# Gustavroot/DeflatedMLMC_Schwinger

Measured on AMD Instinct MI355X. Metric: hutchinson_probe_samples_per_sec_schwinger128, higher is better.
Workload: dtype f64

## Files before the change

deflatedmlmc_schwinger_amd/csrc/sw_engine.hip:

```cpp
#include "../../include/schwinger_hip.h"
#include "sw_kernels.hpp"
#include "sw_pack.hpp"
#include "sw_poly.hpp"

#include <dlfcn.h>

#include <algorithm>
#include <chrono>
#include <cmath>
#include <complex>
#include <cstdarg>
#include <cstdio>
#include <cstdlib>
#include <cstring>
#include <functional>
#include <map>
#include <mutex>
#include <string>
#include <type_traits>
#include <vector>

using swk::cplx;
using swk::cplxf;
using swk::PtrList;
// ... 149 lines not shown
  bool eo_skew_chunk = false;
  bool gram_cycle = true;
  bool eo_product = true;
  int gj_block = 32;
  int eo_tile = 0;
  int dense_lds = 4;
  int eo_tile_dbg = 0;
  int num_cus = 256;
  bool direct_small = true;
  bool lgmres_aug = true;
  bool stencil_nt = false;
  int stencil_tile = 0;
  int stencil_spw = 0;
  bool cgs2 = false;
  bool verify = true;
  bool inner_cgs2 = false;
  bool pyth_last = true;
  bool eo_solve = true;
  bool eo_direct = true;
  bool precond_f32 = false;
  int kd = 0;
  cplx* U = nullptr;
  int defl_gemm = 0;
  int lkd[SW_MAX_LEVELS] = {0};
  cplx* lV[SW_MAX_LEVELS] = {nullptr};
  int* perm_src[SW_MAX_LEVELS] = {nullptr};
  EllOp rhsmap[SW_MAX_LEVELS];
  cplx* partial = nullptr;
  size_t partial_bytes = 0;
  cplx* small = nullptr;
  size_t small_bytes = 0;
  void* stage = nullptr;
  size_t stage_bytes = 0;
  std::vector<std::pair<void*, size_t>> allocs;
  int pb_level = -1, pb_nb = 0, pb_nbp = 0;
  int8_t* pb_probes = nullptr;
  struct ProbeSlot {
    int8_t* p = nullptr;
    size_t bytes = 0;
    int level = -1, nb = 0;
    hipEvent_t ready = nullptr;
    bool pending = false;
  };
  std::vector<ProbeSlot> slots;
  bool mt_set = false;
  uint32_t* mt_win0 = nullptr;
  uint32_t* mt_win = nullptr;
  int mt_cur = 0;
  uint64_t mt_pos = 0;
  uint32_t* mt_poly = nullptr;
  uint64_t mt_dist = 0;
  uint32_t* mt_family = nullptr;
  uint64_t mt_fam_seg = 0;
  int mt_fam_count = 0;
  cplx *pb_x0 = nullptr, *pb_rhs = nullptr, *pb_z = nullptr, *pb_xc = nullptr, *pb_xc2 = nullptr,
       *pb_y = nullptr, *pb_w = nullptr, *pb_w2 = nullptr, *pb_xd = nullptr;
  int pb_ws_nbp = 0;
  cplx* pb_est = nullptr;
  int* pb_iters = nullptr;
  std::vector<int32_t> last_iters_f, last_iters_c;
  bool profiling = false;
  std::vector<EventRec> recs;
  std::vector<hipEvent_t> evpool;
  double tacc[T_NCAT] = {0};
  int64_t tcount[T_NCAT] = {0};
  double twork[T_NCAT] = {0};
  int64_t launches = 0;
  int* d_notconv = nullptr;
  int nc_next = 0;
  int* h_notconv = nullptr;
  int* d_tick = nullptr;
  bool fused_reduce = true;
  double stop_factor = 1.0;
  std::vector<double> direct_relres;
  int64_t direct_fallbacks = 0;
  double alloc_s = 0.0, alloc_bytes = 0.0;
  int64_t alloc_calls = 0, pool_hits = 0;
// ... 34 lines not shown
    field<&sw_engine::mfma_small_tiles>("mfma_small_tiles",
                                        [](double v) { return v == 0.0 || v == 2.0 || v == 4.0; },
                                        "mfma_small_tiles must be 0, 2 or 4"),
    field<&sw_engine::mfma3_tiles>("mfma3_tiles",
                                   [](double v) { const int t = (int)v; return t == 0 || t == 1 || t == 2 || t == 4; },
                                   "mfma3_tiles must be 0, 1, 2 or 4"),
    field<&sw_engine::bsr_map>("bsr_map", [](double v) { return (int)v >= 0 && (int)v <= 3; },
                               "bsr_map must be 0..3"),
    field<&sw_engine::dense_map>("dense_map", [](double v) { return (int)v >= 0 && (int)v <= 3; },
                                 "dense_map must be 0..3"),
    field<&sw_engine::bsr_sub>("bsr_sub", [](double v) { return (int)v >= 1; }, "bsr_sub must be >= 1"),
    field<&sw_engine::bsr_stages>("bsr_stages", [](double v) { return v == 2.0 || v == 4.0 || v == 8.0; },
                                  "bsr_stages must be 2, 4 or 8 (dense_stages: or 16)"),
    field<&sw_engine::dense_stages>("dense_stages",
                                    [](double v) { return v == 2.0 || v == 4.0 || v == 8.0 || v == 16.0; },
                                    "dense_stages must be 2, 4 or 8 (dense_stages: or 16)"),
    field<&sw_engine::bsr_nt>("bsr_nt"),
    field<&sw_engine::bsr_xreg>("bsr_xreg"),
    {"dense_lds", get_field<&sw_engine::dense_lds>,
     [](sw_engine* h, double v) { h->dense_lds = v == 1.0 ? 2 : (int)v; },
     [](double v) { return v == 0.0 || v == 1.0 || v == 2.0 || v == 4.0; }, "dense_lds must be 0, 2 or 4"},
    field<&sw_engine::defl_gemm>("defl_gemm", [](double v) { return v == 0.0 || v == 1.0; },
                                 "defl_gemm must be 0 or 1"),
    field<&sw_engine::fused_reduce>("fused_reduce"),
    {"dot_blocks", [](const sw_engine*) { return (double)g_dot_blocks; },
     [](sw_engine*, double v) { g_dot_blocks = g_dot_pmax = std::max(64, (int)v); }},
    field<&sw_engine::gj_block>("gj_block",
                                [](double v) {
                                  const int b = (int)v;
                                  return b == 0 || (b >= 8 && b <= 256 && b % 8 == 0);
                                },
                                "gj_block must be 0 or a multiple of 8 in 8..256"),
    field<&sw_engine::stencil_nt>("stencil_nt"),
    field<&sw_engine::stencil_tile>("stencil_tile"),
    field<&sw_engine::stencil_spw>("stencil_spw",
                                   [](double v) {
                                     const int t = (int)v;
                                     return t == 0 || t == 1 || t == 2 || t == 4 || t == 8;
                                   },
                                   "stencil_spw must be 0,1,2,4,8"),
    field<&sw_engine::eo_tile>("eo_tile", [](double v) { return v == 0.0 || v == 4.0 || v == 8.0; },
                               "eo_tile must be 0 (off), 4 or 8 waves"),
    {"eo_tile_dbg", get_field<&sw_engine::eo_tile_dbg>, [](sw_engine* h, double v) { h->eo_tile_dbg = (int)v & 3; }},
    field<&sw_engine::eo_skew>("eo_skew", [](double v) { return !(v < -1.0 || v > 65536.0); },
                               "eo_skew must be -1 (automatic), 0 (off) or a strip height"),
    field<&sw_engine::eo_skew_chunk>("eo_skew_chunk"),
// ... 597 lines not shown
  int P, rpb;
  row_blocking(n, nbp, nrm_out != nullptr, &P, &rpb);
  const int ngroups = (P + SW_RED_GROUP - 1) / SW_RED_GROUP;
  if (nrm_out) SWCHK(ensure_partial(h, (size_t)(P + ngroups) * nbp * sizeof(cplx)));
  const bool fused = nrm_out && fused_ok(h, P, nbp);
  const swk::RedArgs ra = red_args(h, fused, P, 1, nbp, nrm_out, nullptr, nullptr);
  const swk::FgTail tl = (fused && tail) ? *tail : kNoTail;
  dim3 grid(P, nbp / 64);
  SWCHK(pick_ge<2, 4, 8, 16, 24, 34>(K, [&](auto KT) {
    if (nrm_out)
      return launch(h, T_AXPY, swk::k_multiaxpy<KT, true, CV, CW>, grid, dim3(SW_BLOCK), V, K, coef, sign, Win, Wout,
                    n, nbp, rpb, h->partial, w32, ra, tl);
    return launch(h, T_AXPY, swk::k_multiaxpy<KT, false, CV, CW>, grid, dim3(SW_BLOCK), V, K, coef, sign, Win, Wout,
                  n, nbp, rpb, h->partial, w32, ra, tl);
  }));
  if (nrm_out && !fused) {
    SWCHK(launch(h, T_DOTS, swk::k_reduce_partials, dim3(1, nbp / 64), dim3(SW_BLOCK), h->partial, P, 1, nbp,
                 nrm_out, (const cplx*)nullptr, (cplx*)nullptr));
  }
  if (tail && !fused) SWCHK(launch_tail(h, *tail));
  return 0;
}

static int zero_vec(sw_engine* h, cplx* p, int n, int nbp) {
  LaunchScope ls(h, T_AXPY);
  HIPCHK(hipMemsetAsync(p, 0, (size_t)n * nbp * sizeof(cplx), h->stream));
  return 0;
}
static int copy_vec(sw_engine* h, cplx* dst, const cplx* src, int n, int nbp) {
  LaunchScope ls(h, T_AXPY);
  HIPCHK(hipMemcpyAsync(dst, src, (size_t)n * nbp * sizeof(cplx), hipMemcpyDeviceToDevice,
                        h->stream));
  return 0;
}

static int ensure_small(sw_engine* h, int nbp) {
  const size_t need = (size_t)(SW_MAX_DEFL + 8) * nbp * sizeof(cplx);
  if (h->small_bytes >= need) return 0;
  if (h->small) SWCHK(dev_free(h, h->small));
  h->small = nullptr;
  void* q;
  SWCHK(dev_alloc(h, &q, need));
  h->small = (cplx*)q;
  h->small_bytes = need;
  return 0;
}
// ... 260 lines not shown
    std::vector<int> ord(P.ngroups);
    if (P.order && h->ell_order)
      HIPCHK(hipMemcpy(ord.data(), P.order, ord.size() * sizeof(int), hipMemcpyDeviceToHost));
    else
      for (int g = 0; g < P.ngroups; ++g) ord[g] = g;
    std::vector<int> ev;
    for (int g : ord) {
      const long long row = (long long)g * P.G;
      const bool even = lv.stencil ? (row < lv.n / 2) : (even_row_tile[row / 16] != 0);
      if (even) ev.push_back(g);
    }
    if (ev.empty()) continue;
    SWCHK(upload(h, &P.order_even, ev.data(), ev.size()));
    P.ngroups_even = (int)ev.size();
  }
  H.even_valid = true;
  return 0;
}

static inline int* sink_slot(sw_engine* h);
static bool f32_capable(const Hier& H, int level);

static int gram_cycle(sw_engine* h, const KrylovSys& sys, const cplx* R, cplx* X, int L, KrylovWS& ws, int nbp,
                      swk::FgTail tg) {
  const size_t vec = (size_t)sys.n * nbp;
  PtrList pu, pz;
  pu.p[0] = R;
  for (int j = 0; j < L; ++j) {
    cplx* z = ws.Z + vec * j;
    cplx* w = ws.V + vec * j;
    SWCHK(sys.precond(pu.p[j], z));
    SWCHK(sys.apply(0, z, nullptr, w));
    pu.p[j + 1] = w;
    pz.p[j] = z;
  }
  tg.kind = SW_TAIL_GRAM;
  tg.s = ws.sc;
  tg.j = L;
  tg.h1 = ws.gram;
  SWCHK(multigram(h, pu, L + 1, sys.n, nbp, ws.gram, &tg));
  return multiaxpy(h, pz, L, ws.sc.ys, 1.0, X, X, sys.n, nbp, nullptr);
}

static int kcycle_gram(sw_engine* h, Hier& H, int level, const cplx* B, cplx* X, int L, KrylovWS& ws, int nbp) {
  swk::FgTail tg{};
  tg.first_cycle = 1;
  tg.notconv = sink_slot(h);
  SWCHK(zero_vec(h, X, H.lv[level].n, nbp));
  return gram_cycle(h, full_system(h, H, level, nbp, true, false), B, X, L, ws, nbp, tg);
}

static int coarse_correction(sw_engine* h, Hier& H, int l, int nbp) {
  Level& lv = H.lv[l];
  Level& lc = H.lv[l + 1];
  const int last = H.nlevels - 1;
  if (lv.kcycle > 0 && l + 1 < last) {
    SWCHK(ensure_krylov(h, lc.kws, lv.kcycle, lc.n, nbp, false));
    int P = 0, rpb = 0;
    row_blocking(lc.n, nbp, true, &P, &rpb);
    if (h->gram_cycle && lv.kcycle <= SW_GRAM_MAXL && fused_ok(h, P, nbp) &&
        !(h->precond_f32 && f32_capable(H, l + 1)))
      return kcycle_gram(h, H, l + 1, lc.b, lc.x, lv.kcycle, lc.kws, nbp);
    return fgmres(h, H, l + 1, lc.b, lc.x, 0.0, lv.kcycle, lv.kcycle, false, lc.kws, nbp, nullptr);
  }
// ... 2245 lines not shown
  }
  return s;
}

static int reduced_rhs(sw_engine* h, Level& lv, const cplx* B, KrylovWS& ws, int nbp) {
  PtrList pl;
  pl.p[0] = B;
  const swk::FgTail tbeg = tail_begin(ws, 1);
  SWCHK(multidot(h, pl, 1, B, lv.n, nbp, ws.nrm, nullptr, nullptr, &tbeg));
  return eo_hop<0>(h, lv, B, B, ws.xacc, nbp);
}

static int fgmres_eo(sw_engine* h, Hier& H, const cplx* B, cplx* X, double tol, int maxiter, int m,
                     KrylovWS& ws, int nbp, int* iters_total) {
  Level& lv = H.lv[0];
  SWCHK(ensure_level_ws(h, lv, nbp));
  SWCHK(reduced_rhs(h, lv, B, ws, nbp));
  SWCHK(fgmres_loop(h, H, 0, reduced_system(h, H, nbp), ws.xacc, X, tol, maxiter, m, true, ws, nbp,
                    iters_total));
  return eo_hop<1>(h, lv, B, X, X, nbp);
}

static int fgmres_eo_gram(sw_engine* h, Hier& H, const cplx* B, cplx* X, double tol, int maxiter, int m,
                          KrylovWS& ws, int nbp, int* iters_total) {
  Level& lv = H.lv[0];
  const int hid_idx = (int)(&H - &h->hier[0]);
  const int hint = h->lazy_sync ? h->sync_hint[hid_idx][0] : 0;
  const KrylovSys sys = reduced_system(h, H, nbp);
  const double tol_stop = tol * h->stop_factor;
  SWCHK(ensure_level_ws(h, lv, nbp));
  SWCHK(reset_slots(h));
  SWCHK(reduced_rhs(h, lv, B, ws, nbp));
  const cplx* bp = ws.xacc;
  SWCHK(zero_vec(h, X, sys.n, nbp));
  std::vector<std::complex<double>> hrr(nbp), hrr0(nbp);
  int done = 0;
  bool converged = false;
  const cplx* Rcur = bp;
  int L = std::min(m, maxiter);
  while (done < maxiter && !converged) {
    L = std::max(1, std::min(L, std::min(m, maxiter - done)));
    int* slot = nullptr;
    SWCHK(take_slot(h, &slot));
    swk::FgTail tg{};
    tg.tol = tol;
    tg.tol_stop = tol_stop;
    tg.iter_base = done;
    tg.notconv = slot;
    SWCHK(gram_cycle(h, sys, Rcur, X, L, ws, nbp, tg));
    done += L;
    SWCHK(sys.apply(1, X, bp, ws.rres));
    Rcur = ws.rres;
    const bool observe = tol_stop > 0.0 && (hint <= 0 || done + m >= hint || done >= maxiter);
    int Lnext = m;
    if (observe) {
      int left = 0;
      SWCHK(read_slot(h, slot, &left));
      if (left == 0) {
        converged = true;
      } else {
        HIPCHK(hipMemcpy(hrr.data(), ws.sc.relres, sizeof(cplx) * nbp, hipMemcpyDeviceToHost));
        HIPCHK(hipMemcpy(hrr0.data(), ws.sc.g, sizeof(cplx) * nbp, hipMemcpyDeviceToHost));
        double need = 1.0;
        for (int c = 0; c < nbp; ++c) {
          const double r1 = hrr[c].real(), r0 = hrr0[c].real();
          if (!(r1 >= tol_stop) || !(r0 > 0.0)) continue;
          const double rate = std::pow(std::min(0.9, std::max(1e-6, r1 / r0)), 1.0 / L);
          need = std::max(need, std::ceil(std::log(0.9 * tol_stop / r1) / std::log(rate)));
        }
        Lnext = (int)std::min<double>(m, need);
      }
    }
    if (converged && h->verify) {
      PtrList pr;
      pr.p[0] = ws.rres;
      int* vslot = nullptr;
      SWCHK(take_slot(h, &vslot));
      const swk::FgTail tv = tail_verify(ws, tol, tol_stop, vslot);
      SWCHK(multidot(h, pr, 1, ws.rres, sys.n, nbp, ws.nrm, nullptr, nullptr, &tv));
      int left = 0;
      SWCHK(read_slot(h, vslot, &left));
      if (left != 0) {
        converged = false;
        Lnext = 1;
      }
    }
    L = Lnext;
  }
  SWCHK(eo_hop<1>(h, lv, B, X, X, nbp));
  if (iters_total) *iters_total = done;
  h->sync_hint[hid_idx][0] = converged ? done : 0;
  return 0;
}

static bool level_is_direct(sw_engine* h, Hier& H, int level) {
  return h->direct_small && level < H.nlevels - 1 && !H.lv[level].stencil && H.lv[level].dinv.set &&
         h->use_mfma;
}

static int solve_dev(sw_engine* h, int hid, int level0, const cplx* B, cplx* X, double tol,
                     int maxiter, int nbp, int* total) {
  Hier& H = h->hier[hid];
  Level& lv = H.lv[level0];
  if (level0 == H.nlevels - 1 && H.nlevels > 1) {
    SWCHK(apply_coarsest(h, H, B, X, nbp));
    if (total) *total = 1;
    return 0;
  }
  if (level_is_direct(h, H, level0)) {
    SWCHK(ensure_level_ws(h, lv, nbp));
    SWCHK(launch_bsr(h, lv.dinv, 0, B, nullptr, X, nbp, T_COARSEST, cplx{0.0, 0.0}));
    SWCHK(apply_op(h, lv, 1, X, B, lv.r, nbp));
    SWCHK(launch_bsr(h, lv.dinv, 0, lv.r, nullptr, lv.t, nbp, T_COARSEST, cplx{0.0, 0.0}));
    SWCHK(vec_add(h, X, lv.t, X, lv.n, nbp));
    if (total) *total = 1;
// ... 4 lines not shown
      SWCHK(dot_into(h, lv.r, lv.r, lv.n, nbp, h->small));
      SWCHK(dot_into(h, B, B, lv.n, nbp, h->small + nbp));
      SWCHK(stream_sync(h));
      std::vector<std::complex<double>> nn(2 * (size_t)nbp);
      HIPCHK(hipMemcpy(nn.data(), h->small, sizeof(cplx) * 2 * nbp, hipMemcpyDeviceToHost));
      double worst = 0.0;
      for (int j = 0; j < nbp; ++j) {
        const double b2 = nn[nbp + j].real(), r2 = nn[j].real();
        const double rr = b2 > 0.0 ? std::sqrt(r2 / b2) : 0.0;
        h->direct_relres[j] = rr;
        worst = std::max(worst, rr);
      }
      if (!(worst > tol * h->stop_factor)) return 0;
      if (pass == 3) break;
      SWCHK(launch_bsr(h, lv.dinv, 0, lv.r, nullptr, lv.t, nbp, T_COARSEST, cplx{0.0, 0.0}));
      SWCHK(vec_add(h, X, lv.t, X, lv.n, nbp));
    }
    h->direct_relres.clear();
    h->direct_fallbacks++;
    const int mfb = std::min(h->restart, std::max(1, maxiter));
    SWCHK(ensure_krylov(h, lv.sws, mfb, lv.n, nbp, true));
    return fgmres(h, H, level0, B, X, tol, maxiter, mfb, true, lv.sws, nbp, total);
  }
  const int m = std::min(h->restart, std::max(1, maxiter));
  SWCHK(ensure_krylov(h, lv.sws, m, lv.n, nbp, true));
  if (eo_solve_eligible(h, H, level0)) {
    const bool k32 = h->precond_f32 && h->f32_krylov && f32_capable(H, 0);
    int P = 0, rpb = 0;
    row_blocking(lv.n / 2, nbp, true, &P, &rpb);
    if (h->gram_cycle && !k32 && m <= SW_GRAM_MAXL && fused_ok(h, P, nbp))
      return fgmres_eo_gram(h, H, B, X, tol, maxiter, m, lv.sws, nbp, total);
    return fgmres_eo(h, H, B, X, tol, maxiter, m, lv.sws, nbp, total);
  }
  return fgmres(h, H, level0, B, X, tol, maxiter, m, true, lv.sws, nbp, total);
}

static int fetch_iters(sw_engine* h, KrylovWS& ws, int nb, int32_t* iters, double* relres,
                       int fallback_iters) {
  std::vector<int> it(ws.nbp);
  std::vector<std::complex<double>> rr(ws.nbp);
  HIPCHK(hipMemcpy(it.data(), ws.sc.iters, sizeof(int) * ws.nbp, hipMemcpyDeviceToHost));
  HIPCHK(hipMemcpy(rr.data(), ws.sc.relres, sizeof(cplx) * ws.nbp, hipMemcpyDeviceToHost));
  for (int j = 0; j < nb; ++j) {
    if (iters) iters[j] = it[j] >= 0 ? it[j] : fallback_iters;
    if (relres) relres[j] = rr[j].real();
  }
  return 0;
}

int sw_solve(sw_engine* h, int hid, int level0, int nb, const double* B, double* X, double tol,
             int maxiter, int32_t* iters, double* relres) {
  SWCHK(check_hier(h, hid, level0, true));
  if (nb <= 0 || !B || !X || maxiter < 1) return sw_fail(h, "bad arguments");
  HIPCHK(hipSetDevice(h->device));
  Hier& H = h->hier[hid];
  const int nbp = pad64(nb);
// ... 8 lines not shown
    for (int j = 0; j < nb; ++j) {
      if (iters) iters[j] = 1;
      if (relres) relres[j] = 0.0;
    }
    return 0;
  }
  if (level_is_direct(h, H, level0) && (int)h->direct_relres.size() >= nb) {
    for (int j = 0; j < nb; ++j) {
      if (iters) iters[j] = 1;
      if (relres) relres[j] = h->direct_relres[j];
    }
    return 0;
  }
  return fetch_iters(h, lv.sws, nb, iters, relres, total);
}

static int ensure_probe_ws(sw_engine* h, int nbp) {
  if (h->pb_ws_nbp == nbp && h->pb_x0) return 0;
  Hier& H0 = h->hier[0];
  int nmax = 0;
  for (int l = 0; l < H0.nlevels; ++l) nmax = std::max(nmax, H0.lv[l].n);
  const size_t cnt = (size_t)nmax * nbp;
  SWCHK(dev_realloc(h, &h->pb_x0, cnt));
  SWCHK(dev_realloc(h, &h->pb_rhs, cnt));
  SWCHK(dev_realloc(h, &h->pb_z, cnt));
  SWCHK(dev_realloc(h, &h->pb_xc, cnt));
  SWCHK(dev_realloc(h, &h->pb_xc2, cnt));
  SWCHK(dev_realloc(h, &h->pb_y, cnt));
  SWCHK(dev_realloc(h, &h->pb_w, cnt));
  SWCHK(dev_realloc(h, &h->pb_w2, cnt));
  SWCHK(dev_realloc(h, &h->pb_xd, cnt));
  SWCHK(dev_realloc(h, &h->pb_est, (size_t)4 * nbp));
  SWCHK(dev_realloc(h, &h->pb_iters, (size_t)2 * nbp));
  h->pb_ws_nbp = nbp;
  return 0;
}

int sw_probes_upload_slot(sw_engine* h, int slot, int level, int nb, const int8_t* probes) {
  SWCHK(check_hier(h, 0, level, true));
  if (nb <= 0 || !probes) return sw_fail(h, "bad arguments");
  if (slot < 0 || slot >= 4096) return sw_fail(h, "probe slot %d out of range", slot);
  HIPCHK(hipSetDevice(h->device));
  Level& lv = h->hier[0].lv[level];
  const size_t bytes = (size_t)nb * lv.n;
  if ((int)h->slots.size() <= slot) h->slots.resize(slot + 1);
  sw_engine::ProbeSlot& sl = h->slots[slot];
// ... 166 lines not shown
  return 0;
}

static int deflate(sw_engine* h, const cplx* U, int kd, const int* srcrow, const cplx* X, cplx* out,
                   int n, int nbp) {
  const int ld = defl_ld(kd);
  cplx* cbuf = h->small + 8 * nbp;
  if (h->defl_gemm || kd > 64) {
    const int nchunks = nbp / 16;
    const int pmax = std::max(1, (n + 63) / 64);
    int P = std::max(1, std::min(pmax, 2048 / nchunks));
    const int rpb = (n + P - 1) / P;
    P = (n + rpb - 1) / rpb;
    SWCHK(ensure_partial(h, (size_t)P * ld * nbp * sizeof(cplx)));
    SWCHK(pick_ge<64, 128, 256>(ld, [&](auto LD) {
      return launch(h, T_DEFL, swk::k_defl_gemm_dots<LD / 64>, dim3(P, nchunks), dim3(SW_BLOCK), U, ld, X, n, nbp,
                    rpb, h->partial);
    }));
    SWCHK(launch(h, T_DEFL, swk::k_reduce_partials, dim3(ld, nbp / 64), dim3(SW_BLOCK), h->partial, P, ld, nbp,
                 cbuf, (const cplx*)nullptr, (cplx*)nullptr));
    return launch(h, T_DEFL, swk::k_defl_gemm_apply, dim3((n + 63) / 64, nbp / 64), dim3(SW_BLOCK), U, ld,
                  (const cplx*)cbuf, srcrow, X, out, n, nbp);
  }
  int P, rpb;
  row_blocking(n, nbp, true, &P, &rpb);
  for (int k0 = 0; k0 < kd; k0 += 32) {
    const int kc = std::min(32, kd - k0);
    SWCHK(ensure_partial(h, (size_t)P * kc * nbp * sizeof(cplx)));
    SWCHK(pick_ge<8, 16, 32>(kc, [&](auto KC) {
      return launch(h, T_DEFL, swk::k_defl_dots<KC>, dim3(P, nbp / 64), dim3(SW_BLOCK), (const cplx*)(U + k0), ld,
                    kc, X, n, nbp, rpb, h->partial);
    }));
    SWCHK(launch(h, T_DEFL, swk::k_reduce_partials, dim3(kc, nbp / 64), dim3(SW_BLOCK), h->partial, P, kc, nbp,
                 cbuf + (size_t)k0 * nbp, (const cplx*)nullptr, (cplx*)nullptr));
  }
  {
    dim3 grid((n + SW_WAVES_PER_BLOCK - 1) / SW_WAVES_PER_BLOCK, nbp / 64);
    SWCHK(launch(h, T_DEFL, swk::k_defl_apply, grid, dim3(SW_BLOCK), U, ld, kd, cbuf, srcrow, X, out, n, nbp));
  }
  return 0;
}

int sw_apply_deflation(sw_engine* h, int which, int level, int nb, const double* X, double* Y) {
  SWCHK(check_hier(h, 0, level, false));
  if (which != 0 && which != 1) return sw_fail(h, "which must be 0 (Hutchinson) or 1 (MLMC level)");
  if (which == 0 && level != 0) return sw_fail(h, "the Hutchinson deflation acts at level 0");
  if (nb <= 0 || !X || !Y) return sw_fail(h, "bad arguments");
  const int kd = which == 0 ? h->kd : h->lkd[level];
  const cplx* U = which == 0 ? h->U : h->lV[level];
  if (kd <= 0 || !U) return sw_fail(h, "no deflation vectors registered at level %d", level);
  HIPCHK(hipSetDevice(h->device));
  Level& lv = h->hier[0].lv[level];
  const int nbp = pad64(nb);
  cplx *a, *b;
  SWCHK(io_vectors(h, lv, nbp, &a, &b));
  SWCHK(ensure_small(h, nbp));
  SWCHK(pack_host(h, lv, nb, X, a, nbp));
  SWCHK(deflate(h, U, kd, which == 0 ? (const int*)h->perm_src[0] : nullptr, a, b, lv.n, nbp));
  return unpack_host(h, lv, nb, b, Y, nbp);
}

int sw_hutch_run(sw_engine* h, int mode, int level, double tol, int maxiter) {
  SWCHK(check_hier(h, 0, level, true));
  if (h->pb_level != level || h->pb_nb <= 0) return sw_fail(h, "no probes uploaded for level %d", level);
  if (maxiter < 1) return sw_fail(h, "maxiter must be >= 1");
  HIPCHK(hipSetDevice(h->device));
  Hier& H0 = h->hier[0];
  const int nb = h->pb_nb, nbp = h->pb_nbp;
  Level& lv = H0.lv[level];
  const int n = lv.n;
  SWCHK(ensure_probe_ws(h, nbp));
  SWCHK(ensure_small(h, nbp));
  if (h->pb_slot >= 0 && h->pb_slot < (int)h->slots.size() && h->slots[h->pb_slot].pending) {
    HIPCHK(hipStreamWaitEvent(h->stream, h->slots[h->pb_slot].ready, 0));
    h->slots[h->pb_slot].pending = false;
  }
  SWCHK(launch(h, T_OTHER, swk::k_pack_i8, dim3((n + 63) / 64, nbp / 64), dim3(SW_BLOCK), h->pb_probes, nb, n,
               (const int*)lv.rowmap, h->pb_x0, nbp));
  const int fine_hid = (level == 0 && h->hier[h->solver_hid].ready) ? h->solver_hid : 0;
  if (fine_hid != 0 && h->hier[fine_hid].lv[0].n != n)
    return sw_fail(h, "solver hierarchy level-0 size mismatch");
  if (mode == SW_MODE_HUTCHINSON) {
    if (level != 0) return sw_fail(h, "Hutchinson mode runs at level 0");
    const int kd = h->kd;
    if (kd > 0) {
      SWCHK(deflate(h, h->U, kd, (const int*)h->perm_src[0], h->pb_x0, h->pb_rhs, n, nbp));
    } else {
      dim3 grid((n + SW_WAVES_PER_BLOCK - 1) / SW_WAVES_PER_BLOCK, nbp / 64);
      SWCHK(launch(h, T_DEFL, swk::k_gather_rows, grid, dim3(SW_BLOCK), (const int*)h->perm_src[0], h->pb_x0,
                   h->pb_rhs, n, nbp));
    }
    int total = 0;
    SWCHK(solve_dev(h, fine_hid, 0, h->pb_rhs, h->pb_z, tol, maxiter, nbp, &total));
    SWCHK(dot_into(h, h->pb_x0, h->pb_z, n, nbp, h->pb_est));
    SWCHK(stream_sync(h));
    SWCHK(record_iters(h, &h->hier[fine_hid].lv[0].sws, total, h->last_iters_f, nb));
    h->last_iters_c.assign(nb, 0);
    return 0;
  }
  if (mode == SW_MODE_LEVEL) {
    const cplx* xdef = h->pb_x0;
    if (h->rhsmap[level].set) {
      SWCHK(launch_ell(h, h->rhsmap[level], 0, xdef, nullptr, h->pb_rhs, nbp, T_OTHER));
      xdef = h->pb_rhs;
// ... 275 lines not shown
```

deflatedmlmc_schwinger_amd/csrc/sw_kernels.hpp:

```cpp
#pragma once
#include <hip/hip_runtime.h>
#include <stdint.h>

namespace swk {

typedef double2 cplx;

#define SW_WAVE 64
#define SW_BLOCK 256
#define SW_WAVES_PER_BLOCK 4

__device__ __forceinline__ cplx cmake(double a, double b) { cplx r; r.x = a; r.y = b; return r; }
__device__ __forceinline__ cplx cadd(cplx a, cplx b) { return cmake(a.x + b.x, a.y + b.y); }
__device__ __forceinline__ cplx csub(cplx a, cplx b) { return cmake(a.x - b.x, a.y - b.y); }
__device__ __forceinline__ cplx cmul(cplx a, cplx b) {
  return cmake(fma(a.x, b.x, -a.y * b.y), fma(a.x, b.y, a.y * b.x));
}
__device__ __forceinline__ cplx cmulc(cplx a, cplx b) {
  return cmake(fma(a.x, b.x, a.y * b.y), fma(a.x, b.y, -a.y * b.x));
}
__device__ __forceinline__ void cfma(cplx& acc, cplx a, cplx b) {
  acc.x = fma(a.x, b.x, acc.x);
  acc.x = fma(-a.y, b.y, acc.x);
  acc.y = fma(a.x, b.y, acc.y);
// ... 1404 lines not shown
  const size_t item = (size_t)blockIdx.x * SW_WAVES_PER_BLOCK + (threadIdx.x >> 6);
  if (item >= (size_t)(n >> 4) * KS) return;
  const int rt = (int)(item / KS), ks = (int)(item - (size_t)rt * KS);
  const cplx v = A[((size_t)rt * 16 + (lane & 15)) * n + k0 + 4 * ks + (lane >> 4)];
  vals[item * 64 + lane] = cmake(-v.x, -v.y);
  if (lane == 0) kcol[item] = 4 * ks;
}

__global__ __launch_bounds__(SW_BLOCK) void k_gj_unpermute(cplx* __restrict__ A, int n,
                                                           const int* __restrict__ pivs) {
  const int r = blockIdx.x * SW_BLOCK + threadIdx.x;
  if (r >= n) return;
  cplx* row = A + (size_t)r * n;
  for (int k = n - 1; k >= 0; --k) {
    const int p = pivs[k];
    if (p != k) {
      const cplx t = row[k];
      row[k] = row[p];
      row[p] = t;
    }
  }
}

__global__ __launch_bounds__(SW_BLOCK) void k_pack_i8(const int8_t* __restrict__ src, int nb,
                                                      int n, const int* __restrict__ rowmap,
                                                      cplx* __restrict__ dst, int nbp) {
  __shared__ int8_t tile[64][65];
  const int i0 = blockIdx.x * 64;
  const int j0 = blockIdx.y * 64;
  const int tx = threadIdx.x & 63, ty = threadIdx.x >> 6;
  for (int jj = ty; jj < 64; jj += 4) {
    const int j = j0 + jj, i = i0 + tx;
    tile[jj][tx] = (j < nb && i < n) ? src[(size_t)j * n + i] : (int8_t)0;
  }
  __syncthreads();
  for (int ii = ty; ii < 64; ii += 4) {
    const int i = i0 + ii;
    if (i < n) {
      const size_t row = rowmap ? (size_t)rowmap[i] : (size_t)i;
      const int v = tile[tx][ii];
      dst[row * nbp + j0 + tx] = (v == 2 || v == -2) ? cmake(0.0, (double)(v / 2)) : cmake((double)v, 0.0);
    }
  }
}

__global__ __launch_bounds__(SW_BLOCK) void k_pack_c(const cplx* __restrict__ src, int nb, int n,
                                                     const int* __restrict__ rowmap,
                                                     cplx* __restrict__ dst, int nbp) {
  __shared__ cplx tile[64][65];
  const int i0 = blockIdx.x * 64;
  const int j0 = blockIdx.y * 64;
  const int tx = threadIdx.x & 63, ty = threadIdx.x >> 6;
  for (int jj = ty; jj < 64; jj += 4) {
    const int j = j0 + jj, i = i0 + tx;
    tile[jj][tx] = (j < nb && i < n) ? src[(size_t)j * n + i] : cmake(0.0, 0.0);
  }
  __syncthreads();
  for (int ii = ty; ii < 64; ii += 4) {
    const int i = i0 + ii;
    if (i < n) {
      const size_t row = rowmap ? (size_t)rowmap[i] : (size_t)i;
      dst[row * nbp + j0 + tx] = tile[tx][ii];
    }
  }
}

// ... 653 lines not shown
                                                        int rows_per_block,
                                                        cplx* __restrict__ partial,
                                                        cplxf* __restrict__ W32, RedArgs ra, FgTail tail) {
  __shared__ double redn[3][64];
  __shared__ cplx redt[NORM ? 256 : 1];
  const int wave = threadIdx.x >> 6, lane = threadIdx.x & 63;
  const size_t col = (size_t)blockIdx.y * 64 + lane;
  const int r0 = blockIdx.x * rows_per_block;
  const int r1 = min(n, r0 + rows_per_block);
  cplx c[KT];
#pragma unroll
  for (int k = 0; k < KT; ++k) {
    c[k] = cmake(0.0, 0.0);
    if (k < K) {
      const cplx t = coef[(size_t)k * nbp + col];
      c[k] = cmake(sign * t.x, sign * t.y);
    }
  }
  double nrm = 0.0;
  constexpr int UNR = (sizeof(CV) == sizeof(cplxf) && sizeof(CW) == sizeof(cplxf)) ? 4 : 2;
#pragma unroll UNR
  for (int r = r0 + wave; r < r1; r += SW_WAVES_PER_BLOCK) {
    const size_t off = (size_t)r * nbp + col;
    cplx w = widen(Win[off]);
#pragma unroll
    for (int k = 0; k < KT; ++k)
      if (k < K) cfma(w, c[k], widen(V.p[k][off]));
    Wout[off] = narrow<CW>(w);
    if (W32) W32[off] = cmake((float)w.x, (float)w.y);
    if (NORM) nrm = fma(w.x, w.x, fma(w.y, w.y, nrm));
  }
  if (NORM) {
    if (wave > 0) redn[wave - 1][lane] = nrm;
    __syncthreads();
    if (wave == 0) {
      nrm += redn[0][lane];
      nrm += redn[1][lane];
      nrm += redn[2][lane];
      st_partial(&partial[(size_t)blockIdx.x * nbp + col], cmake(nrm, 0.0), ra.tick1 != nullptr);
    }
    if (ra.tick1) reduce_and_tail<1>(partial, 1, nbp, ra, tail, redt);
  }
}

__global__ __launch_bounds__(SW_BLOCK) void k_mr_update(const cplx* __restrict__ alpha,
                                                        cplx* __restrict__ X, cplx* __restrict__ R,
                                                        const cplx* __restrict__ T, int n, int nbp,
// ... 20 lines not shown
  size_t i = (size_t)blockIdx.x * blockDim.x + threadIdx.x;
  const size_t stride = (size_t)gridDim.x * blockDim.x;
  for (; i < count; i += stride) dst[i] = cmul(w, src[i]);
}

__global__ __launch_bounds__(SW_BLOCK) void k_add(const cplx* __restrict__ a, const cplx* __restrict__ b,
                                                  cplx* __restrict__ dst, size_t count) {
  size_t i = (size_t)blockIdx.x * blockDim.x + threadIdx.x;
  const size_t stride = (size_t)gridDim.x * blockDim.x;
  for (; i < count; i += stride) dst[i] = cadd(a[i], b[i]);
}

__global__ __launch_bounds__(SW_BLOCK) void k_gather_rows(const int* __restrict__ srcrow,
                                                          const cplx* __restrict__ src,
                                                          cplx* __restrict__ dst, int n, int nbp) {
  const int wave = threadIdx.x >> 6, lane = threadIdx.x & 63;
  const size_t col = (size_t)blockIdx.y * 64 + lane;
  const int r = blockIdx.x * SW_WAVES_PER_BLOCK + wave;
  if (r >= n) return;
  const int s = srcrow ? srcrow[r] : r;
  dst[(size_t)r * nbp + col] = src[(size_t)s * nbp + col];
}

template <int KT>
__global__ __launch_bounds__(SW_BLOCK) void k_defl_dots(const cplx* __restrict__ U, int ldu,
                                                        int kd, const cplx* __restrict__ X, int n,
                                                        int nbp, int rows_per_block,
                                                        cplx* __restrict__ partial) {
  __shared__ cplx red[3][8][64];
  const int wave = threadIdx.x >> 6, lane = threadIdx.x & 63;
  const size_t col = (size_t)blockIdx.y * 64 + lane;
  const int r0 = blockIdx.x * rows_per_block;
  const int r1 = min(n, r0 + rows_per_block);
  cplx acc[KT];
#pragma unroll
  for (int k = 0; k < KT; ++k) acc[k] = cmake(0.0, 0.0);
  for (int r = r0 + wave; r < r1; r += SW_WAVES_PER_BLOCK) {
    const int ru = __builtin_amdgcn_readfirstlane(r);
    const cplx x = X[(size_t)ru * nbp + col];
    const cplx* u = U + (size_t)ru * ldu;
#pragma unroll
    for (int k = 0; k < KT; ++k)
      if (k < kd) cfmac(acc[k], u[k], x);
  }
  for (int kb = 0; kb < KT; kb += 8) {
    if (kb >= kd) break;
    if (wave > 0) {
#pragma unroll
      for (int k = 0; k < 8; ++k)
        if (kb + k < KT) red[wave - 1][k][lane] = acc[kb + k];
    }
    __syncthreads();
    if (wave == 0) {
#pragma unroll
      for (int k = 0; k < 8; ++k) {
        if (kb + k < KT && kb + k < kd) {
          cplx s = acc[kb + k];
          s = cadd(s, red[0][k][lane]);
          s = cadd(s, red[1][k][lane]);
          s = cadd(s, red[2][k][lane]);
          partial[((size_t)blockIdx.x * kd + kb + k) * nbp + col] = s;
        }
// ... 1 lines not shown
    }
    __syncthreads();
  }
}

__global__ __launch_bounds__(SW_BLOCK) void k_defl_apply(const cplx* __restrict__ U, int ldu, int kd,
                                                         const cplx* __restrict__ c,
                                                         const int* __restrict__ srcrow,
                                                         const cplx* __restrict__ X,
                                                         cplx* __restrict__ out, int n, int nbp) {
  const int wave = threadIdx.x >> 6, lane = threadIdx.x & 63;
  const size_t col = (size_t)blockIdx.y * 64 + lane;
  const int r = __builtin_amdgcn_readfirstlane(blockIdx.x * SW_WAVES_PER_BLOCK + wave);
  if (r >= n) return;
  const int s = srcrow ? srcrow[r] : r;
  cplx x = X[(size_t)s * nbp + col];
  const cplx* u = U + (size_t)s * ldu;
#pragma unroll 4
  for (int k = 0; k < kd; ++k) {
    const cplx ck = c[(size_t)k * nbp + col];
    cfma(x, cmake(-u[k].x, -u[k].y), ck);
  }
  out[(size_t)r * nbp + col] = x;
}

template <int KT>
__global__ __launch_bounds__(SW_BLOCK) void k_defl_gemm_dots(const cplx* __restrict__ U, int ldu,
                                                             const cplx* __restrict__ X, int n, int nbp,
                                                             int rows_per_block,
                                                             cplx* __restrict__ partial) {
  const int lane = threadIdx.x & 63, wave = threadIdx.x >> 6;
  const int k = lane >> 4, c = lane & 15;
  const int t0 = wave * KT;
  const int nt = min(KT, ldu / 16 - t0);
  if (nt <= 0) return;
  const int r0 = blockIdx.x * rows_per_block;
  const int r1 = min(n, r0 + rows_per_block);
  const size_t j = (size_t)blockIdx.y * 16 + c;
  sw_double4 cr[KT], ci[KT];
#pragma unroll
  for (int t = 0; t < KT; ++t) cr[t] = ci[t] = sw_double4{0.0, 0.0, 0.0, 0.0};
  for (int row = r0 + k; row < r1 + k; row += 4) {
    const bool in = row < r1;
    const cplx x = in ? X[(size_t)row * nbp + j] : cmake(0.0, 0.0);
    const cplx* up = U + (size_t)row * ldu + t0 * 16 + c;
#pragma unroll
// ... 428 lines not shown
```

Before: 35970.

## Fuse Hutchinson probe pipeline into int8 probe, deflated-RHS and estimate kernels

Adds a fused Hutchinson path for the fine level. It keeps the probes as int8 rows instead of expanding them to complex f64, computes the deflation dots straight from the int8 data, and builds the even-odd reduced RHS with the deflation projection inside one stencil kernel, which also produces the norm. The final reconstruction and the trace dot product are merged into a single estimate kernel, and the GMRES start skips the zero-fill and the x-accumulate read. This is meant to remove several full-vector passes and kernel launches per batch, at the cost of a specialised code path that only applies under narrower eligibility conditions.

```diff
diff --git a/deflatedmlmc_schwinger_amd/csrc/sw_engine.hip b/deflatedmlmc_schwinger_amd/csrc/sw_engine.hip
--- a/deflatedmlmc_schwinger_amd/csrc/sw_engine.hip
+++ b/deflatedmlmc_schwinger_amd/csrc/sw_engine.hip
@@ -195,6 +195,7 @@
   int kd = 0;
   cplx* U = nullptr;
   int defl_gemm = 0;
+  int batch_fused = 1;
   int lkd[SW_MAX_LEVELS] = {0};
   cplx* lV[SW_MAX_LEVELS] = {nullptr};
   int* perm_src[SW_MAX_LEVELS] = {nullptr};
@@ -226,6 +227,7 @@
   uint32_t* mt_family = nullptr;
   uint64_t mt_fam_seg = 0;
   int mt_fam_count = 0;
+  int8_t* pb_rows8 = nullptr;
   cplx *pb_x0 = nullptr, *pb_rhs = nullptr, *pb_z = nullptr, *pb_xc = nullptr, *pb_xc2 = nullptr,
        *pb_y = nullptr, *pb_w = nullptr, *pb_w2 = nullptr, *pb_xd = nullptr;
   int pb_ws_nbp = 0;
@@ -306,6 +308,8 @@
      [](double v) { return v == 0.0 || v == 1.0 || v == 2.0 || v == 4.0; }, "dense_lds must be 0, 2 or 4"},
     field<&sw_engine::defl_gemm>("defl_gemm", [](double v) { return v == 0.0 || v == 1.0; },
                                  "defl_gemm must be 0 or 1"),
+    field<&sw_engine::batch_fused>("batch_fused", [](double v) { return v == 0.0 || v == 1.0; },
+                                   "batch_fused must be 0 or 1"),
     field<&sw_engine::fused_reduce>("fused_reduce"),
     {"dot_blocks", [](const sw_engine*) { return (double)g_dot_blocks; },
      [](sw_engine*, double v) { g_dot_blocks = g_dot_pmax = std::max(64, (int)v); }},
@@ -949,6 +953,24 @@
   return 0;
 }
 
+template <class CX>
+static int defl_dots(sw_engine* h, const cplx* U, int kd, const CX* X, int n, int nbp, cplx* cbuf) {
+  const int ld = defl_ld(kd);
+  int P, rpb;
+  row_blocking(n, nbp, true, &P, &rpb);
+  for (int k0 = 0; k0 < kd; k0 += 32) {
+    const int kc = std::min(32, kd - k0);
+    SWCHK(ensure_partial(h, (size_t)P * kc * nbp * sizeof(cplx)));
+    SWCHK(pick_ge<8, 16, 32>(kc, [&](auto KC) {
+      return launch(h, T_DEFL, swk::k_defl_dots<KC, CX>, dim3(P, nbp / 64), dim3(SW_BLOCK), (const cplx*)(U + k0),
+                    ld, kc, X, n, nbp, rpb, h->partial);
+    }));
+    SWCHK(launch(h, T_DEFL, swk::k_reduce_partials, dim3(kc, nbp / 64), dim3(SW_BLOCK), h->partial, P, kc, nbp,
+                 cbuf + (size_t)k0 * nbp, (const cplx*)nullptr, (cplx*)nullptr));
+  }
+  return 0;
+}
+
 static int zero_vec(sw_engine* h, cplx* p, int n, int nbp) {
   LaunchScope ls(h, T_AXPY);
   HIPCHK(hipMemsetAsync(p, 0, (size_t)n * nbp * sizeof(cplx), h->stream));
@@ -1255,7 +1277,7 @@
 static bool f32_capable(const Hier& H, int level);
 
 static int gram_cycle(sw_engine* h, const KrylovSys& sys, const cplx* R, cplx* X, int L, KrylovWS& ws, int nbp,
-                      swk::FgTail tg) {
+                      swk::FgTail tg, bool x_zero = false) {
   const size_t vec = (size_t)sys.n * nbp;
   PtrList pu, pz;
   pu.p[0] = R;
@@ -1272,7 +1294,7 @@
   tg.j = L;
   tg.h1 = ws.gram;
   SWCHK(multigram(h, pu, L + 1, sys.n, nbp, ws.gram, &tg));
-  return multiaxpy(h, pz, L, ws.sc.ys, 1.0, X, X, sys.n, nbp, nullptr);
+  return multiaxpy(h, pz, L, ws.sc.ys, 1.0, x_zero ? (const cplx*)nullptr : X, X, sys.n, nbp, nullptr);
 }
 
 static int kcycle_gram(sw_engine* h, Hier& H, int level, const cplx* B, cplx* X, int L, KrylovWS& ws, int nbp) {
@@ -3564,7 +3586,7 @@
 }
 
 static int fgmres_eo_gram(sw_engine* h, Hier& H, const cplx* B, cplx* X, double tol, int maxiter, int m,
-                          KrylovWS& ws, int nbp, int* iters_total) {
+                          KrylovWS& ws, int nbp, int* iters_total, bool rhs_ready = false) {
   Level& lv = H.lv[0];
   const int hid_idx = (int)(&H - &h->hier[0]);
   const int hint = h->lazy_sync ? h->sync_hint[hid_idx][0] : 0;
@@ -3572,9 +3594,11 @@
   const double tol_stop = tol * h->stop_factor;
   SWCHK(ensure_level_ws(h, lv, nbp));
   SWCHK(reset_slots(h));
-  SWCHK(reduced_rhs(h, lv, B, ws, nbp));
+  if (!rhs_ready) {
+    SWCHK(reduced_rhs(h, lv, B, ws, nbp));
+    SWCHK(zero_vec(h, X, sys.n, nbp));
+  }
   const cplx* bp = ws.xacc;
-  SWCHK(zero_vec(h, X, sys.n, nbp));
   std::vector<std::complex<double>> hrr(nbp), hrr0(nbp);
   int done = 0;
   bool converged = false;
@@ -3589,7 +3613,7 @@
     tg.tol_stop = tol_stop;
     tg.iter_base = done;
     tg.notconv = slot;
-    SWCHK(gram_cycle(h, sys, Rcur, X, L, ws, nbp, tg));
+    SWCHK(gram_cycle(h, sys, Rcur, X, L, ws, nbp, tg, rhs_ready && done == 0));
     done += L;
     SWCHK(sys.apply(1, X, bp, ws.rres));
     Rcur = ws.rres;
@@ -3629,10 +3653,20 @@
     }
     L = Lnext;
   }
-  SWCHK(eo_hop<1>(h, lv, B, X, X, nbp));
+  if (!rhs_ready) SWCHK(eo_hop<1>(h, lv, B, X, X, nbp));
   if (iters_total) *iters_total = done;
   h->sync_hint[hid_idx][0] = converged ? done : 0;
   return 0;
+}
+
+static int outer_restart(sw_engine* h, int maxiter) { return std::min(h->restart, std::max(1, maxiter)); }
+
+static bool eo_gram_eligible(sw_engine* h, Hier& H, int level, int m, int nbp) {
+  if (!eo_solve_eligible(h, H, level)) return false;
+  const bool k32 = h->precond_f32 && h->f32_krylov && f32_capable(H, 0);
+  int P = 0, rpb = 0;
+  row_blocking(H.lv[0].n / 2, nbp, true, &P, &rpb);
+  return h->gram_cycle && !k32 && m <= SW_GRAM_MAXL && fused_ok(h, P, nbp);
 }
 
 static bool level_is_direct(sw_engine* h, Hier& H, int level) {
@@ -3683,16 +3717,11 @@
     SWCHK(ensure_krylov(h, lv.sws, mfb, lv.n, nbp, true));
     return fgmres(h, H, level0, B, X, tol, maxiter, mfb, true, lv.sws, nbp, total);
   }
-  const int m = std::min(h->restart, std::max(1, maxiter));
+  const int m = outer_restart(h, maxiter);
   SWCHK(ensure_krylov(h, lv.sws, m, lv.n, nbp, true));
-  if (eo_solve_eligible(h, H, level0)) {
-    const bool k32 = h->precond_f32 && h->f32_krylov && f32_capable(H, 0);
-    int P = 0, rpb = 0;
-    row_blocking(lv.n / 2, nbp, true, &P, &rpb);
-    if (h->gram_cycle && !k32 && m <= SW_GRAM_MAXL && fused_ok(h, P, nbp))
-      return fgmres_eo_gram(h, H, B, X, tol, maxiter, m, lv.sws, nbp, total);
-    return fgmres_eo(h, H, B, X, tol, maxiter, m, lv.sws, nbp, total);
-  }
+  if (eo_gram_eligible(h, H, level0, m, nbp))
+    return fgmres_eo_gram(h, H, B, X, tol, maxiter, m, lv.sws, nbp, total);
+  if (eo_solve_eligible(h, H, level0)) return fgmres_eo(h, H, B, X, tol, maxiter, m, lv.sws, nbp, total);
   return fgmres(h, H, level0, B, X, tol, maxiter, m, true, lv.sws, nbp, total);
 }
 
@@ -3747,6 +3776,7 @@
   for (int l = 0; l < H0.nlevels; ++l) nmax = std::max(nmax, H0.lv[l].n);
   const size_t cnt = (size_t)nmax * nbp;
   SWCHK(dev_realloc(h, &h->pb_x0, cnt));
+  SWCHK(dev_realloc(h, &h->pb_rows8, cnt));
   SWCHK(dev_realloc(h, &h->pb_rhs, cnt));
   SWCHK(dev_realloc(h, &h->pb_z, cnt));
   SWCHK(dev_realloc(h, &h->pb_xc, cnt));
@@ -3959,18 +3989,7 @@
     return launch(h, T_DEFL, swk::k_defl_gemm_apply, dim3((n + 63) / 64, nbp / 64), dim3(SW_BLOCK), U, ld,
                   (const cplx*)cbuf, srcrow, X, out, n, nbp);
   }
-  int P, rpb;
-  row_blocking(n, nbp, true, &P, &rpb);
-  for (int k0 = 0; k0 < kd; k0 += 32) {
-    const int kc = std::min(32, kd - k0);
-    SWCHK(ensure_partial(h, (size_t)P * kc * nbp * sizeof(cplx)));
-    SWCHK(pick_ge<8, 16, 32>(kc, [&](auto KC) {
-      return launch(h, T_DEFL, swk::k_defl_dots<KC>, dim3(P, nbp / 64), dim3(SW_BLOCK), (const cplx*)(U + k0), ld,
-                    kc, X, n, nbp, rpb, h->partial);
-    }));
-    SWCHK(launch(h, T_DEFL, swk::k_reduce_partials, dim3(kc, nbp / 64), dim3(SW_BLOCK), h->partial, P, kc, nbp,
-                 cbuf + (size_t)k0 * nbp, (const cplx*)nullptr, (cplx*)nullptr));
-  }
+  SWCHK(defl_dots(h, U, kd, X, n, nbp, cbuf));
   {
     dim3 grid((n + SW_WAVES_PER_BLOCK - 1) / SW_WAVES_PER_BLOCK, nbp / 64);
     SWCHK(launch(h, T_DEFL, swk::k_defl_apply, grid, dim3(SW_BLOCK), U, ld, kd, cbuf, srcrow, X, out, n, nbp));
@@ -3997,6 +4016,57 @@
   return unpack_host(h, lv, nb, b, Y, nbp);
 }
 
+static void pair_blocking(int Vh, int* P, int* ppb) {
+  *ppb = ((Vh + 2047) / 2048 + SW_WAVES_PER_BLOCK - 1) / SW_WAVES_PER_BLOCK * SW_WAVES_PER_BLOCK;
+  *P = (Vh + *ppb - 1) / *ppb;
+}
+static bool hutch_fused_eligible(sw_engine* h, Hier& H, int maxiter, int nbp) {
+  if (!h->batch_fused || h->defl_gemm || h->kd > 32) return false;
+  if (!eo_gram_eligible(h, H, 0, outer_restart(h, maxiter), nbp)) return false;
+  const Level& lv = H.lv[0];
+  int P, ppb;
+  pair_blocking(lv.L * lv.L / 2, &P, &ppb);
+  return lv.n == 2 * lv.L * lv.L && fused_ok(h, P, nbp);
+}
+
+static int hutch_run_fused(sw_engine* h, Hier& H, double tol, int maxiter) {
+  Level& lv = H.lv[0];
+  const int nb = h->pb_nb, nbp = h->pb_nbp, n = lv.n, kd = h->kd;
+  const int m = outer_restart(h, maxiter);
+  KrylovWS& ws = lv.sws;
+  SWCHK(ensure_krylov(h, ws, m, n, nbp, true));
+  SWCHK(launch(h, T_DEFL, swk::k_probe_rows_i8, dim3((n + 63) / 64, nbp / 64), dim3(SW_BLOCK), h->pb_probes, nb, n,
+               (const int*)h->hier[0].lv[0].rowmap, h->pb_rows8, nbp));
+  cplx* cbuf = h->small + 8 * nbp;
+  if (kd > 0) SWCHK(defl_dots(h, h->U, kd, (const int8_t*)h->pb_rows8, n, nbp, cbuf));
+  const swk::StencilArgs a = stencil_args<cplx>(h, lv, nbp, true);
+  const double di = 1.0 / a.diag;
+  int P, ppb;
+  pair_blocking(a.Vh, &P, &ppb);
+  const int ngroups = (P + SW_RED_GROUP - 1) / SW_RED_GROUP;
+  SWCHK(ensure_partial(h, (size_t)(P + ngroups) * nbp * sizeof(cplx)));
+  {
+    swk::HutchProbes g{};
+    g.x0 = h->pb_rows8;
+    g.U = h->U;
+    g.ldu = kd > 0 ? defl_ld(kd) : 0;
+    g.kd = kd;
+    g.c = cbuf;
+    g.srcrow = h->perm_src[0];
+    SWCHK(launch(h, T_DEFL, swk::k_hutch_rhs, dim3(P, nbp / 64), dim3(SW_BLOCK), g, a, di, h->pb_rhs, ws.xacc, ppb,
+                 h->partial, red_args(h, true, P, 1, nbp, ws.nrm, nullptr, nullptr), tail_begin(ws, 1)));
+  }
+  int total = 0;
+  SWCHK(fgmres_eo_gram(h, H, h->pb_rhs, h->pb_z, tol, maxiter, m, ws, nbp, &total, true));
+  SWCHK(launch(h, T_DOTS, swk::k_hutch_est, dim3(P, nbp / 64), dim3(SW_BLOCK), (const int8_t*)h->pb_rows8,
+               (const cplx*)h->pb_rhs, (const cplx*)h->pb_z, a, di, ppb, h->partial,
+               red_args(h, true, P, 1, nbp, h->pb_est, nullptr, nullptr)));
+  SWCHK(stream_sync(h));
+  SWCHK(record_iters(h, &ws, total, h->last_iters_f, nb));
+  h->last_iters_c.assign(nb, 0);
+  return 0;
+}
+
 int sw_hutch_run(sw_engine* h, int mode, int level, double tol, int maxiter) {
   SWCHK(check_hier(h, 0, level, true));
   if (h->pb_level != level || h->pb_nb <= 0) return sw_fail(h, "no probes uploaded for level %d", level);
@@ -4012,11 +4082,13 @@
     HIPCHK(hipStreamWaitEvent(h->stream, h->slots[h->pb_slot].ready, 0));
     h->slots[h->pb_slot].pending = false;
   }
-  SWCHK(launch(h, T_OTHER, swk::k_pack_i8, dim3((n + 63) / 64, nbp / 64), dim3(SW_BLOCK), h->pb_probes, nb, n,
-               (const int*)lv.rowmap, h->pb_x0, nbp));
   const int fine_hid = (level == 0 && h->hier[h->solver_hid].ready) ? h->solver_hid : 0;
   if (fine_hid != 0 && h->hier[fine_hid].lv[0].n != n)
     return sw_fail(h, "solver hierarchy level-0 size mismatch");
+  if (mode == SW_MODE_HUTCHINSON && level == 0 && hutch_fused_eligible(h, h->hier[fine_hid], maxiter, nbp))
+    return hutch_run_fused(h, h->hier[fine_hid], tol, maxiter);
+  SWCHK(launch(h, T_OTHER, swk::k_pack_i8, dim3((n + 63) / 64, nbp / 64), dim3(SW_BLOCK), h->pb_probes, nb, n,
+               (const int*)lv.rowmap, h->pb_x0, nbp));
   if (mode == SW_MODE_HUTCHINSON) {
     if (level != 0) return sw_fail(h, "Hutchinson mode runs at level 0");
     const int kd = h->kd;
diff --git a/deflatedmlmc_schwinger_amd/csrc/sw_kernels.hpp b/deflatedmlmc_schwinger_amd/csrc/sw_kernels.hpp
--- a/deflatedmlmc_schwinger_amd/csrc/sw_kernels.hpp
+++ b/deflatedmlmc_schwinger_amd/csrc/sw_kernels.hpp
@@ -1450,9 +1450,17 @@
   }
 }
 
-__global__ __launch_bounds__(SW_BLOCK) void k_pack_i8(const int8_t* __restrict__ src, int nb,
-                                                      int n, const int* __restrict__ rowmap,
-                                                      cplx* __restrict__ dst, int nbp) {
+__device__ __forceinline__ cplx probe_decode(int v) {
+  return (v == 2 || v == -2) ? cmake(0.0, (double)(v / 2)) : cmake((double)v, 0.0);
+}
+__device__ __forceinline__ cplx probe_load(cplx v) { return v; }
+__device__ __forceinline__ cplx probe_load(int8_t v) { return probe_decode(v); }
+__device__ __forceinline__ void probe_store(cplx* p, int v) { *p = probe_decode(v); }
+__device__ __forceinline__ void probe_store(int8_t* p, int v) { *p = (int8_t)v; }
+
+template <class O>
+__device__ __forceinline__ void pack_i8_tile(const int8_t* __restrict__ src, int nb, int n,
+                                             const int* __restrict__ rowmap, O* __restrict__ dst, int nbp) {
   __shared__ int8_t tile[64][65];
   const int i0 = blockIdx.x * 64;
   const int j0 = blockIdx.y * 64;
@@ -1466,10 +1474,19 @@
     const int i = i0 + ii;
     if (i < n) {
       const size_t row = rowmap ? (size_t)rowmap[i] : (size_t)i;
-      const int v = tile[tx][ii];
-      dst[row * nbp + j0 + tx] = (v == 2 || v == -2) ? cmake(0.0, (double)(v / 2)) : cmake((double)v, 0.0);
-    }
-  }
+      probe_store(&dst[row * nbp + j0 + tx], tile[tx][ii]);
+    }
+  }
+}
+__global__ __launch_bounds__(SW_BLOCK) void k_pack_i8(const int8_t* __restrict__ src, int nb,
+                                                      int n, const int* __restrict__ rowmap,
+                                                      cplx* __restrict__ dst, int nbp) {
+  pack_i8_tile(src, nb, n, rowmap, dst, nbp);
+}
+__global__ __launch_bounds__(SW_BLOCK) void k_probe_rows_i8(const int8_t* __restrict__ src, int nb,
+                                                            int n, const int* __restrict__ rowmap,
+                                                            int8_t* __restrict__ dst, int nbp) {
+  pack_i8_tile(src, nb, n, rowmap, dst, nbp);
 }
 
 __global__ __launch_bounds__(SW_BLOCK) void k_pack_c(const cplx* __restrict__ src, int nb, int n,
@@ -2169,7 +2186,7 @@
 #pragma unroll UNR
   for (int r = r0 + wave; r < r1; r += SW_WAVES_PER_BLOCK) {
     const size_t off = (size_t)r * nbp + col;
-    cplx w = widen(Win[off]);
+    cplx w = Win ? widen(Win[off]) : cmake(0.0, 0.0);
 #pragma unroll
     for (int k = 0; k < KT; ++k)
       if (k < K) cfma(w, c[k], widen(V.p[k][off]));
@@ -2236,9 +2253,9 @@
   dst[(size_t)r * nbp + col] = src[(size_t)s * nbp + col];
 }
 
-template <int KT>
+template <int KT, class CX = cplx>
 __global__ __launch_bounds__(SW_BLOCK) void k_defl_dots(const cplx* __restrict__ U, int ldu,
-                                                        int kd, const cplx* __restrict__ X, int n,
+                                                        int kd, const CX* __restrict__ X, int n,
                                                         int nbp, int rows_per_block,
                                                         cplx* __restrict__ partial) {
   __shared__ cplx red[3][8][64];
@@ -2251,7 +2268,7 @@
   for (int k = 0; k < KT; ++k) acc[k] = cmake(0.0, 0.0);
   for (int r = r0 + wave; r < r1; r += SW_WAVES_PER_BLOCK) {
     const int ru = __builtin_amdgcn_readfirstlane(r);
-    const cplx x = X[(size_t)ru * nbp + col];
+    const cplx x = probe_load(X[(size_t)ru * nbp + col]);
     const cplx* u = U + (size_t)ru * ldu;
 #pragma unroll
     for (int k = 0; k < KT; ++k)
@@ -2299,6 +2316,134 @@
     cfma(x, cmake(-u[k].x, -u[k].y), ck);
   }
   out[(size_t)r * nbp + col] = x;
+}
+
+struct HutchProbes {
+  const int8_t* x0;
+  const cplx* U;
+  int ldu, kd;
+  const cplx* c;
+  const int* srcrow;
+};
+
+template <int NR>
+__device__ __forceinline__ void hutch_rhs_rows(const HutchProbes& g, const int (&row)[NR], size_t col, int nbp,
+                                               cplx (&v)[NR]) {
+  const cplx* u[NR];
+#pragma unroll
+  for (int i = 0; i < NR; ++i) {
+    const int s = g.srcrow ? g.srcrow[row[i]] : row[i];
+    v[i] = probe_decode(g.x0[(size_t)s * nbp + col]);
+    u[i] = g.U + (size_t)s * g.ldu;
+  }
+#pragma unroll 2
+  for (int k = 0; k < g.kd; ++k) {
+    const cplx ck = g.c[(size_t)k * nbp + col];
+#pragma unroll
+    for (int i = 0; i < NR; ++i) cfma(v[i], cmake(-u[i][k].x, -u[i][k].y), ck);
+  }
+}
+
+__device__ __forceinline__ void pair_site(int sh, int q, int L, int& x, int& y) {
+  const int hl = L >> 1;
+  y = sh / hl;
+  x = 2 * (sh - y * hl) + ((q + y) & 1);
+}
+
+__device__ __forceinline__ void block_sum_reduce(cplx v, cplx* __restrict__ partial, int nbp, const RedArgs& ra,
+                                                 const FgTail& tail) {
+  __shared__ cplx redw[3][64];
+  __shared__ cplx redt[256];
+  const int wave = threadIdx.x >> 6, lane = threadIdx.x & 63;
+  if (wave > 0) redw[wave - 1][lane] = v;
+  __syncthreads();
+  if (wave == 0) {
+    v = cadd(v, redw[0][lane]);
+    v = cadd(v, redw[1][lane]);
+    v = cadd(v, redw[2][lane]);
+    st_partial(&partial[(size_t)blockIdx.x * nbp + (size_t)blockIdx.y * 64 + lane], v, true);
+  }
+  reduce_and_tail<1>(partial, 1, nbp, ra, tail, redt);
+}
+
+__global__ __launch_bounds__(SW_BLOCK) void k_hutch_rhs(HutchProbes g, StencilArgs a, double beta,
+                                                        cplx* __restrict__ rhs, cplx* __restrict__ bpe,
+                                                        int pairs_per_block, cplx* __restrict__ partial,
+                                                        RedArgs ra, FgTail tail) {
+  const int wave = threadIdx.x >> 6, lane = threadIdx.x & 63;
+  const size_t col = (size_t)blockIdx.y * 64 + lane;
+  const int L = a.L, Vh = a.Vh, nbp = a.nbp;
+  const int p0 = blockIdx.x * pairs_per_block;
+  const int p1 = min(Vh, p0 + pairs_per_block);
+  double nrm = 0.0;
+  for (int shv = p0 + wave; shv < p1; shv += SW_WAVES_PER_BLOCK) {
+    const int sh = __builtin_amdgcn_readfirstlane(shv);
+    int x, y;
+    pair_site(sh, 0, L, x, y);
+    const int xp = wrap_p(x, L), xm = wrap_m(x, L), yp = wrap_p(y, L), ym = wrap_m(y, L);
+    const int re = 2 * sh;
+    const int rxp = (int)eo_row(xp, y, L, Vh), rxm = (int)eo_row(xm, y, L, Vh);
+    const int ryp = (int)eo_row(x, yp, L, Vh), rym = (int)eo_row(x, ym, L, Vh);
+    const int rows[10] = {re, re + 1, rxp, rxp + 1, rxm, rxm + 1, ryp, ryp + 1, rym, rym + 1};
+    cplx v[10];
+    hutch_rhs_rows<10>(g, rows, col, nbp, v);
+    Site2 acc;
+    acc.s0 = cmake(0.0, 0.0);
+    acc.s1 = acc.s0;
+    hop_acc<0>(acc, a.U1[y * L + x], Site2{v[2], v[3]});
+    hop_acc<1>(acc, a.U1[y * L + xm], Site2{v[4], v[5]});
+    hop_acc<2>(acc, a.U2[y * L + x], Site2{v[6], v[7]});
+    hop_acc<3>(acc, a.U2[ym * L + x], Site2{v[8], v[9]});
+    bpe[(size_t)re * nbp + col] = clin(1.0, v[0], beta, acc.s0);
+    bpe[(size_t)(re + 1) * nbp + col] = clin(1.0, v[1], beta, acc.s1);
+    const int ro = 2 * (Vh + sh);
+    const int rowo[2] = {ro, ro + 1};
+    cplx w[2];
+    hutch_rhs_rows<2>(g, rowo, col, nbp, w);
+    rhs[(size_t)ro * nbp + col] = w[0];
+    rhs[(size_t)(ro + 1) * nbp + col] = w[1];
+    nrm = fma(v[0].x, v[0].x, fma(v[0].y, v[0].y, nrm));
+    nrm = fma(v[1].x, v[1].x, fma(v[1].y, v[1].y, nrm));
+    nrm = fma(w[0].x, w[0].x, fma(w[0].y, w[0].y, nrm));
+    nrm = fma(w[1].x, w[1].x, fma(w[1].y, w[1].y, nrm));
+  }
+  block_sum_reduce(cmake(nrm, 0.0), partial, nbp, ra, tail);
+}
+
+__global__ __launch_bounds__(SW_BLOCK) void k_hutch_est(const int8_t* __restrict__ x0,
+                                                        const cplx* __restrict__ B,
+                                                        const cplx* __restrict__ X, StencilArgs a, double di,
+                                                        int pairs_per_block, cplx* __restrict__ partial,
+                                                        RedArgs ra) {
+  const int wave = threadIdx.x >> 6, lane = threadIdx.x & 63;
+  const size_t col = (size_t)blockIdx.y * 64 + lane;
+  const int L = a.L, Vh = a.Vh, nbp = a.nbp;
+  const int p0 = blockIdx.x * pairs_per_block;
+  const int p1 = min(Vh, p0 + pairs_per_block);
+  const cplx* S = X + col;
+  cplx e = cmake(0.0, 0.0);
+  for (int shv = p0 + wave; shv < p1; shv += SW_WAVES_PER_BLOCK) {
+    const int sh = __builtin_amdgcn_readfirstlane(shv);
+    const size_t re = (size_t)2 * sh * nbp + col;
+    cfmac(e, probe_decode(x0[re]), X[re]);
+    cfmac(e, probe_decode(x0[re + nbp]), X[re + nbp]);
+    int x, y;
+    pair_site(sh, 1, L, x, y);
+    const int xp = wrap_p(x, L), xm = wrap_m(x, L), yp = wrap_p(y, L), ym = wrap_m(y, L);
+    Site2 acc;
+    acc.s0 = cmake(0.0, 0.0);
+    acc.s1 = acc.s0;
+    hop_acc<0>(acc, a.U1[y * L + x], ld_site(S, xp, y, L, Vh, nbp));
+    hop_acc<1>(acc, a.U1[y * L + xm], ld_site(S, xm, y, L, Vh, nbp));
+    hop_acc<2>(acc, a.U2[y * L + x], ld_site(S, x, yp, L, Vh, nbp));
+    hop_acc<3>(acc, a.U2[ym * L + x], ld_site(S, x, ym, L, Vh, nbp));
+    const size_t ro = (size_t)2 * (Vh + sh) * nbp + col;
+    cfmac(e, probe_decode(x0[ro]), clin(di, B[ro], di, acc.s0));
+    cfmac(e, probe_decode(x0[ro + nbp]), clin(di, B[ro + nbp], di, acc.s1));
+  }
+  FgTail none{};
+  none.kind = SW_TAIL_NONE;
+  block_sum_reduce(e, partial, nbp, ra, none);
 }
 
 template <int KT>
```

Result: no change. 36180 (median of 6 runs) (+0.6%).
